# zhiyuns/AFCM

Measured on AMD Instinct MI355X. Metric: generator fwd+bwd images/sec @256^2, higher is better.
Workload: dtype bf16; 1 GPU; AFCM --model stylegan3 generator training step (fwd + L1 loss + bwd + grad all-reduce + Adam), IXI T1->T2 shape: 256x256, 4->1 channels, full-width 58.5M-param generator, random init; global_batch=16, per_gpu_batch=16, resolution=256, parallelism=dp1, world_size=1, gradient_buckets=0, comm_dtype=fp32, homogeneous_dot=True

## Files before the change

afcm_amd/_lib.py:

```python
import ctypes as C
import os

import torch

_HERE = os.path.dirname(os.path.abspath(__file__))
LIB_PATH = os.environ.get('AFCM_HIP_LIB') or os.path.join(_HERE, 'libafcm_hip.so')

F32, F16, BF16 = 0, 1, 2
E_NOKERNEL, E_INVALID = -1, -2
SIGNS_NONE, SIGNS_WRITE, SIGNS_READ = 0, 1, 2

_DTYPES = {torch.float32: F32, torch.float16: F16, torch.bfloat16: BF16}


class FilteredLReluArgs(C.Structure):
    _fields_ = [
        ('x', C.c_void_p), ('y', C.c_void_p), ('b', C.c_void_p), ('signs', C.c_void_p),
        ('fu', C.c_void_p), ('fd', C.c_void_p),
        ('dtype', C.c_int32),
        ('n', C.c_int32), ('c', C.c_int32), ('xh', C.c_int32), ('xw', C.c_int32), ('yh', C.c_int32), ('yw', C.c_int32),
        ('fuw', C.c_int32), ('fuh', C.c_int32), ('fdw', C.c_int32), ('fdh', C.c_int32),
        ('up', C.c_int32), ('down', C.c_int32),
        ('px0', C.c_int32), ('px1', C.c_int32), ('py0', C.c_int32), ('py1', C.c_int32),
        ('sx', C.c_int32), ('sy', C.c_int32), ('sh', C.c_int32), ('swb', C.c_int32),
# ... 48 lines not shown
    'afcm_filtered_lrelu': (C.c_int, [C.POINTER(FilteredLReluArgs), _vp]),
    'afcm_filtered_lrelu_workspace_bytes': (C.c_int64, []),
    'afcm_filtered_lrelu_prepare': (C.c_int, [C.POINTER(FilteredLReluArgs), _vp]),
    'afcm_filtered_lrelu_act': (C.c_int, [_vp, _vp, _i32, _i32, _i32, _i32, _i32, _i32, _i32, _i32, _i32, _f32, _f32, _f32, _i32, _vp]),
    'afcm_upfirdn2d': (C.c_int, [_vp, _vp, _vp, _i32, _i32, _i32, _i32, _i32, _i32, _i32, _i32, _i32, _i32, _i32, _i32, _i32,
                                 _i32, _i32, _i32, _f32, _vp]),
    'afcm_bias_act': (C.c_int, [_vp, _vp, _vp, _vp, _vp, _vp, _i32, _i64, _i64, _i32, _i32, _i32, _f32, _f32, _f32, _vp]),
    'afcm_conv2d_block_k': (C.c_int, [_i32]),
    'afcm_conv2d_block_k_ks': (C.c_int, [_i32, _i32]),
    'afcm_conv2d_pack_weights_bk': (C.c_int, [_vp, _vp, _i32, _i32, _i32, _i32, _i32, _i32, _i32, _vp]),
    'afcm_conv2d_pack_weights': (C.c_int, [_vp, _vp, _i32, _i32, _i32, _i32, _i32, _i32, _vp]),
    'afcm_conv2d_pack_weights2': (C.c_int, [_vp, _vp, _vp, _i32, _i32, _i32, _i32, _i32, _i32, _vp]),
    'afcm_conv2d': (C.c_int, [_vp, _vp, _vp, _vp, _vp, _i32, _i32, _i32, _i32, _i32, _i32, _i32, _i32, _i32, _vp]),
    'afcm_conv2d_ld': (C.c_int, [_vp, _vp, _vp, _vp, _vp, _i32, _i32, _i32, _i32, _i32, _i32, _i32, _i32, _i32, _i32, _i32, _vp]),
    'afcm_conv2d_plan': (C.c_int, [_i32] * 11 + [C.POINTER(_i32)]),
    'afcm_conv2d_wgrad_plan': (C.c_int, [_i32] * 11 + [C.POINTER(_i32)]),
    'afcm_conv2d_wgrad_splits': (C.c_int, [_i32, _i32, _i32, _i32]),
    'afcm_conv2d_wgrad': (C.c_int, [_vp, _vp, _vp, _vp, _i32, _i32, _i32, _i32, _i32, _i32, _i32, _i32, _vp]),
    'afcm_conv2d_wgrad_ld': (C.c_int, [_vp, _vp, _vp, _vp, _i32, _i32, _i32, _i32, _i32, _i32, _i32, _i32, _i32, _i32, _vp]),
    'afcm_conv2d_wgrad_dots_ld': (C.c_int, [_vp, _vp, _vp, _vp, _vp, _vp, _i32, _i32, _i32, _i32, _i32, _i32, _i32, _i32, _i32, _i32, _vp]),
    'afcm_scale_planes': (C.c_int, [_vp, _vp, _vp, _i32, _i32, _i64, _i32, _vp]),
    'afcm_plane_dot': (C.c_int, [_vp, _vp, _vp, _i32, _i64, _i32, _vp]),
    'afcm_plane_dot_ld': (C.c_int, [_vp, _vp, _vp, _i32, _i64, _i32, _i32, _i32, _i32, _vp]),
    'afcm_split16': (C.c_int, [_vp, _vp, _vp, _vp, _i32, _i64, _i32, _i32, _i64, _vp]),
    'afcm_conv2d_split': (C.c_int, [_vp, _vp, _vp, _vp, _vp, _i32, _i32, _i32, _i32, _i32, _i32, _i32, _i32, _i32, C.c_uint32, _i64, _vp, _vp, _vp]),
    'afcm_amax_bits': (C.c_int, [_vp, _vp, _i64, _i32, _vp, _vp]),
    'afcm_unscale': (C.c_int, [_vp, _i64, _vp, _vp, _vp]),
    'afcm_plane_dot_parts': (C.c_int, [_vp, _vp, _i64, _i32, _vp, _i32, _i64, _i32, _vp, _vp]),
    'afcm_conv2d_pack_split': (C.c_int, [_vp, _vp, _vp, _i32, _i32, _i32, _i32, _i32, _i32, C.c_uint32, _vp]),
    'afcm_plane_dot_gated_ld': (C.c_int, [_vp, _vp, _vp, _i32, _i64, _i32, _i32, _i32, _i32, _vp, _i32, _vp, _vp, _vp, _vp, _vp]),
# ... 86 lines not shown
```

afcm_amd/csrc/conv2d.hip:

```cpp
#include <stdlib.h>
#include <string.h>

#include <type_traits>

#include "conv2d_common.h"
#include "flrelu_mfma_common.h"

namespace afcm {

template <typename T> struct ConvCfg;
template <> struct ConvCfg<bf16_t> { static constexpr int BK = 16, PITCH = 24; };
template <> struct ConvCfg<f16_t>  { static constexpr int BK = 16, PITCH = 24; };
template <> struct ConvCfg<float>  { static constexpr int BK = 8,  PITCH = 9;  };

static inline int conv_bk(int dtype, int ks);
int conv2d_direct_small_cin(const void* x, void* y, const void* wp, const float* oscale, const float* obias, int dtype, int n, int cin, int cout,
                            int h, int w, int pad, int rows_pad, int bk, int ldx, int ldy, hipStream_t st);

constexpr int kPatchMax = 416;
constexpr int kPlaneX16 = 416;
constexpr int kPatchMaxX16 = kPlaneX16 - 4;
constexpr int kPatchMaxS2 = 704;
constexpr int kSlots = 256;

// ... 2 lines not shown
    void* y;
    const void* wp;
    const float* oscale;
    const float* obias;
    int N, Cin, Cout, H, W, P, Q;
    int ldx, ldy;
    int pad;
    int TH, TW, PWL, tilesX, tilesY;
    int Opad, nkc;
    int total_blocks;
    int o_base;
    unsigned magicTW;
    unsigned magicTX, magicTY, magicN, magicPC;
    int nkc_real; unsigned magicNK, term_parts; int part_bytes, last_part_bytes;
    const unsigned* bound_a; const unsigned* bound_b;
};

__host__ __device__ inline unsigned magic_u32(unsigned d) { return (unsigned)((0x100000000ull + d - 1) / d); }
__device__ __forceinline__ unsigned udiv_magic(unsigned n, unsigned magic) { return magic ? __umulhi(n, magic) : n; }

template <typename T, int BM_O, int KS>
__global__ __launch_bounds__(256, (sizeof(T) == 4 ? 1 : 2)) void conv2d_fwd_kernel(ConvParams p) {
    typedef ConvCfg<T> C;
    constexpr int BK = C::BK, PITCH = C::PITCH, MI = BM_O / 64, KK = KS * KS;
    constexpr bool F32 = sizeof(T) == 4;
    constexpr int EPV = 16 / sizeof(T);
    constexpr int PPR = BK / EPV;
    constexpr int NPIECES = KK * BM_O * PPR;
    constexpr int NWP = cdiv(NPIECES, 256);
    __shared__ __attribute__((aligned(16))) T lds[(KK * BM_O + kPatchMax) * PITCH];
// ... 213 lines not shown
            for (int reg = 0; reg < 16; reg++) ob[reg] = p.obias[min(obase + (reg & 3) + 8 * (reg >> 2), p.Cout - 1)];
        }
#pragma unroll
        for (int reg = 0; reg < 16; reg++) {
            const int o = obase + (reg & 3) + 8 * (reg >> 2);
            if (o < p.Cout) {
                T* yo = yn + (size_t)o * pq;
#pragma unroll
                for (int ti = 0; ti < 4; ti++)
                    if (poff[ti] >= 0) yo[poff[ti]] = from_f32<T>(acc[mi][ti][reg] * sc[reg] + ob[reg]);
            }
        }
    }
}

template <typename T, int BM_O, bool SPLIT = false, bool FASTEPI = false>
__global__ __launch_bounds__(256, 2) void conv2d_fwd16x_kernel(ConvParams p) {
    static_assert(sizeof(T) == 2, "16-bit types only");
    static_assert(!(SPLIT && FASTEPI), "the fp32-output epilogue has no fast form");
    typedef typename std::conditional<SPLIT, float, T>::type TO;
    constexpr int KS = 3, KK = 9, BK = 32, MO = BM_O / 32, NT = 8, BRING = MO == 4 ? 4 : 3;
    constexpr int ARING = MO == 2 ? 6 : 9;
    static_assert((KK * MO) % ARING == 0 && ARING >= 2 * MO, "static slots; a tap's fragments and the next tap's are live together");
    constexpr int PLANE_B = kPlaneX16 * 16;
    constexpr int BUF_B = 4 * PLANE_B;
    static_assert(PLANE_B % 256 == 0 && kPatchMaxX16 % 4 == 0, "planes: a multiple of 256 bytes apart, patch + sink inside");
    typedef typename std::conditional<std::is_same<T, bf16_t>::value, bf16x8, f16x8>::type frag_t;
    typedef __attribute__((ext_vector_type(4))) float f32x4;
    typedef __attribute__((ext_vector_type(4))) unsigned u32x4;
    typedef __attribute__((ext_vector_type(2))) unsigned u32x2;
    __shared__ __attribute__((aligned(256))) unsigned char lds[2 * BUF_B];

    const int tid = threadIdx.x, lane = tid & 63;
    const int wave = __builtin_amdgcn_readfirstlane(tid >> 6);
// ... 222 lines not shown
                if (has_sc) sc[mo] = __builtin_bit_cast(f32x4, __builtin_amdgcn_raw_buffer_load_b128(srs, sboff, 0, 0));
                if (has_ob) ob[mo] = __builtin_bit_cast(f32x4, __builtin_amdgcn_raw_buffer_load_b128(brs, sboff, 0, 0));
            }
            const int i16 = lane_e & 15, chalf = (lane_e >> 4) & 1, hh = lane_e >> 5;
            const int q4 = i16 >> 2, p4 = i16 & 3;
            unsigned rd_off[2];
#pragma unroll
            for (int r = 0; r < 2; r++) {
                const int prw = 8 * hh + 4 * r + q4;
                rd_off[r] = prw * EROW + (((chalf * 4 + p4) ^ ((prw >> 1) & 7)) << 3);
            }
            unsigned wr_off[2];
#pragma unroll
            for (int k = 0; k < 2; k++) wr_off[k] = (unsigned)(c16e * EROW + (((4 * k + ge) ^ ((c16e >> 1) & 7)) << 3));
            unsigned gbyte[8], gfullm = 0, slow_any = 0;
#pragma unroll
            for (int it = 0; it < (FASTEPI ? 0 : 8); it++) {
                const int j0 = wpx * 128 + (2 * it + hh) * 8;
                const int gpy = (int)__umulhi((unsigned)j0, p.magicTW), gpx = j0 - gpy * p.TW;
                const int gy = y0 + gpy, gx = x0 + gpx;
                const bool in_tile = j0 < p.TH * p.TW && gy < p.P;
                const bool valid = in_tile && gx < p.Q;
                const bool straddle = gpx + 8 > p.TW;
                const bool slow = in_tile && (straddle || (valid && gx + 8 > p.ldy));
                gbyte[it] = valid ? (unsigned)((gy * p.ldy + gx) * 2) : kGOut;
                if (!slow) gfullm |= 1u << it;
                if (__builtin_amdgcn_ballot_w64(slow) != 0) slow_any |= 1u << it;
            }
#pragma unroll
            for (int mi = 0; mi < (MO + 1) / 2; mi++) {
                const int rowbase = o0 + wo * (BM_O / 2) + mi * 32;
                const int o = rowbase + chalf * 16 + i16;
                const unsigned obyte = (o < p.Cout && mi * 32 + chalf * 16 < BM_O / 2) ? (unsigned)(o * pq * 2) : kOOut;
#pragma unroll
                for (int half = 0; half < 2; half++) {
#pragma unroll
                    for (int k = 0; k < 2; k++) {
                        const int mo = 2 * mi + k;
                        if (mo >= MO) continue;
#pragma unroll
                        for (int t4 = 0; t4 < 4; t4++) {
                            const int ti = 4 * half + t4;
                            uint2 w;
                            w.x = pack2<T>(acc[mo][ti][0] * sc[mo][0] + ob[mo][0], acc[mo][ti][1] * sc[mo][1] + ob[mo][1]);
                            w.y = pack2<T>(acc[mo][ti][2] * sc[mo][2] + ob[mo][2], acc[mo][ti][3] * sc[mo][3] + ob[mo][3]);
                            *(uint2*)(ebuf + wr_off[k] + t4 * (16 * EROW)) = w;
                        }
                    }
#pragma unroll
                    for (int i4 = 0; i4 < 4; i4++) {
                        const int it = 4 * half + i4;
                        union { s16x4 v[2]; eu32x4 q; } u;
#pragma unroll
                        for (int r = 0; r < 2; r++)
                            u.v[r] = __builtin_amdgcn_ds_read_tr16_b64_v4i16((__attribute__((address_space(3))) s16x4*)(ebuf + i4 * (16 * EROW) + rd_off[r]));
                        if constexpr (FASTEPI) {
                            const int b16 = wpx * 128 + 16 * it;
                            const int gpy = (int)__umulhi((unsigned)b16, p.magicTW), gpxs = b16 - gpy * p.TW;
                            const int gy = y0 + gpy, gxs = x0 + gpxs;
                            if (b16 < p.TH * p.TW && gy < p.P && gxs < p.Q) {
                                unsigned vo = obyte + 16u * (unsigned)hh;
                                if (gxs + 8 >= p.Q && hh) vo = kGOut;
                                __builtin_amdgcn_raw_buffer_store_b128(u.q, yrs, vo, (gy * p.ldy + gxs) * 2, 0);
                            }
                            continue;
                        }
                        const bool full = (gfullm >> it) & 1;
                        __builtin_amdgcn_raw_buffer_store_b128(u.q, yrs, full ? obyte + gbyte[it] : kGOut, 0, 0);
                        if ((slow_any >> it) & 1) {
                            if (!full) {
// ... 579 lines not shown
    }
    if (!split && x16 && rows_pad % 128 == 64 && rows_pad > 128) {
        pl.family = kConv128p64; pl.rows = 64; pl.big = rows_pad / 128;
        pl.items = tiles;
        pl.grid = conv_persistent_grid(pl.items, 3);
        return pl;
    }
    pl.family = small ? kConv64 : kConv128; pl.rows = small ? 64 : 128;
    pl.items = tiles * cdiv(cout, pl.rows);
    pl.grid = (small && (split || x16)) ? conv_persistent_grid(pl.items, 3) : pl.items;
    return pl;
}

template <typename T, int BM_O, bool SPLIT>
static int launch_fwd16x(const ConvParams& p, dim3 grid, bool fast, hipStream_t st) {
    if (!SPLIT && fast) hipLaunchKernelGGL((conv2d_fwd16x_kernel<T, BM_O, false, true>), grid, dim3(256), 0, st, p);
    else hipLaunchKernelGGL((conv2d_fwd16x_kernel<T, BM_O, SPLIT>), grid, dim3(256), 0, st, p);
    return hip_status(hipGetLastError());
}

static ConvParams conv_params(void* y, const void* x, const void* wp, const float* oscale, const float* obias, int n, int cin, int cout,
                              int h, int w, int P, int Q, int pad, int ldx, int ldy, int TH, int TW, int PWL, int rows_pad, int nkc) {
    ConvParams p;
    p.x = x; p.y = y; p.wp = wp; p.oscale = oscale; p.obias = obias;
    p.N = n; p.Cin = cin; p.Cout = cout; p.H = h; p.W = w;
    p.P = P; p.Q = Q;
    p.pad = pad;
    p.ldx = ldx; p.ldy = ldy;
    p.TH = TH; p.TW = TW; p.PWL = PWL;
    p.tilesX = cdiv(p.Q, p.TW); p.tilesY = cdiv(p.P, p.TH);
    p.magicTW = (unsigned)((0x100000000ull + (unsigned)p.TW - 1) / (unsigned)p.TW);
    p.magicTX = magic_u32((unsigned)p.tilesX); p.magicTY = magic_u32((unsigned)p.tilesY); p.magicN = magic_u32((unsigned)p.N); p.magicPC = magic_u32((unsigned)(p.PWL >> 2));
    p.Opad = rows_pad;
    p.nkc = nkc;
    p.nkc_real = p.nkc; p.magicNK = 0; p.term_parts = 0; p.part_bytes = 0; p.last_part_bytes = 0; p.bound_a = p.bound_b = nullptr; p.total_blocks = 0; p.o_base = 0;
    return p;
}

template <typename T, int BM_O>
static int launch_conv(ConvParams p, int ks, hipStream_t st, long long blocks, long long pgrid, bool fast, int o_base = 0) {
    p.o_base = o_base;
    AFCM_REQUIRE(blocks > 0 && blocks < (1ll << 31), "conv2d: grid of %lld blocks is out of range", blocks);
    dim3 grid((unsigned)blocks), block(256);
    p.total_blocks = (int)blocks;
    if constexpr (sizeof(T) == 2) {
        if (ks == 3) return launch_fwd16x<T, BM_O, false>(p, BM_O == 64 ? dim3((unsigned)pgrid) : grid, fast, st);
        hipLaunchKernelGGL((conv2d_fwd_kernel<T, BM_O, 1>), grid, block, 0, st, p);
    } else {
        if (ks == 3) hipLaunchKernelGGL((conv2d_fwd_kernel<T, BM_O, 3>), grid, block, 0, st, p);
        else hipLaunchKernelGGL((conv2d_fwd_kernel<T, BM_O, 1>), grid, block, 0, st, p);
    }
    return hip_status(hipGetLastError());
}

}

using namespace afcm;

extern "C" int afcm_conv2d_block_k(int32_t dtype) { return dtype == AFCM_F32 ? ConvCfg<float>::BK : ConvCfg<bf16_t>::BK; }
static inline int afcm::conv_bk(int dtype, int ks) { return (dtype != AFCM_F32 && ks == 3) ? 32 : afcm_conv2d_block_k(dtype); }
extern "C" int afcm_conv2d_block_k_ks(int32_t dtype, int32_t ks) { return conv_bk(dtype, ks); }

template <typename T>
static void launch_pack8(void* dst0, void* dst1, const float* w, int cout, int cin, int ks, int rows_pad0, int rows_pad1, int BK, hipStream_t st) {
    const int omax = dst0 ? rows_pad0 : round_up(cout, BK), imax = dst1 ? rows_pad1 : round_up(cin, BK);
    constexpr int BKT = ConvCfg<T>::BK;
    const int ti = BK > 16 ? PackTile<32>::TI : PackTile<BKT>::TI, to = BK > 16 ? PackTile<32>::TO : PackTile<BKT>::TO;
    dim3 grid((unsigned)cdiv(imax > cin ? imax : cin, ti), (unsigned)cdiv(omax > cout ? omax : cout, to)), block(256);
// ... 109 lines not shown
    AFCM_REQUIRE(blocks > 0 && blocks < (1ll << 31), "conv2d_stride2: grid of %lld blocks is out of range", blocks);
    AFCM_REQUIRE((long long)cin * h * w * 2ll < (1ll << 31), "conv2d_stride2: image out of range");
    if (dtype == AFCM_F16) hipLaunchKernelGGL((conv2d_fwd16s2_kernel<f16_t, 128>), dim3((unsigned)blocks), dim3(256), 0, (hipStream_t)stream, p);
    else hipLaunchKernelGGL((conv2d_fwd16s2_kernel<bf16_t, 128>), dim3((unsigned)blocks), dim3(256), 0, (hipStream_t)stream, p);
    return hip_status(hipGetLastError());
}

extern "C" int afcm_conv2d(void* y, const void* x, const void* wpacked, const float* oscale, const float* obias, int32_t dtype, int32_t n,
                           int32_t cin, int32_t cout, int32_t h, int32_t w, int32_t ks, int32_t pad, int32_t rows_pad, void* stream) {
    return afcm_conv2d_ld(y, x, wpacked, oscale, obias, dtype, n, cin, cout, h, w, ks, pad, rows_pad, 0, 0, stream);
}

extern "C" int afcm_conv2d_ld(void* y, const void* x, const void* wpacked, const float* oscale, const float* obias, int32_t dtype, int32_t n,
                              int32_t cin, int32_t cout, int32_t h, int32_t w, int32_t ks, int32_t pad, int32_t rows_pad, int32_t x_pitch,
                              int32_t y_pitch, void* stream) {
    AFCM_REQUIRE(y != nullptr && x != nullptr && wpacked != nullptr, "conv2d: null pointer");
    AFCM_REQUIRE(dtype == AFCM_F32 || dtype == AFCM_F16 || dtype == AFCM_BF16, "x must be float32, float16 or bfloat16");
    AFCM_REQUIRE(n > 0 && cin > 0 && cout > 0 && h > 0 && w > 0, "x is empty");
    AFCM_REQUIRE(ks == 1 || ks == 3, "only 1x1 and 3x3 kernels are supported");
    AFCM_REQUIRE(pad >= 0 && pad <= ks - 1, "padding must be in [0, k-1]");
    AFCM_REQUIRE(dtype == AFCM_F32 || (w % 2 == 0), "16-bit conv2d needs an even input width (got %d)", w);
    AFCM_REQUIRE(rows_pad >= cout && rows_pad % 64 == 0, "rows_pad must be a multiple of 64 covering cout");
    const int P = h + 2 * pad - ks + 1, Q = w + 2 * pad - ks + 1;
    AFCM_REQUIRE(P >= 1 && Q >= 1, "output must be at least 1x1");
    const int ldx = x_pitch ? x_pitch : w, ldy = y_pitch ? y_pitch : Q;
    if (ldx != w || ldy != Q) {
        AFCM_REQUIRE(dtype != AFCM_F32 && ks == 3, "conv2d: row pitches need the 16-bit 3x3 kernel");
        AFCM_REQUIRE(ldx >= w && ldy >= Q && ((ldx | ldy) & 1) == 0, "conv2d: row pitches %d / %d must be even and cover the widths %d / %d", ldx, ldy, w, Q);
        AFCM_REQUIRE((long long)cout * P * ldy < (1ll << 30), "conv2d: pitched output image is out of range");
    }
    AFCM_REQUIRE(dtype == AFCM_F32 || ks != 3 || (long long)cout * P * ldy * 2 < (1ll << 30), "conv2d: 16-bit output image of %lld bytes is out of range (< 2^30)", (long long)cout * P * ldy * 2);
    const ConvPlan pl = conv_plan(dtype, n, cin, cout, P, Q, ks, rows_pad, ldy, false);
    if (pl.family == kConvDirect)
        return conv2d_direct_small_cin(x, y, wpacked, oscale, obias, dtype, n, cin, cout, h, w, pad, rows_pad, 32, ldx, ldy, (hipStream_t)stream);
    ConvParams p = conv_params(y, x, wpacked, oscale, obias, n, cin, cout, h, w, P, Q, pad, ldx, ldy, pl.TH, pl.TW, pl.PWL, rows_pad, cdiv(cin, conv_bk(dtype, ks)));
    hipStream_t st = (hipStream_t)stream;
    if (pl.family == kConv96) {
        AFCM_REQUIRE(pl.items > 0 && pl.items < (1ll << 31), "conv2d: grid of %lld blocks is out of range", pl.items);
        p.total_blocks = (int)pl.items;
        const dim3 g96((unsigned)pl.grid);
        return dtype == AFCM_F16 ? launch_fwd16x<f16_t, 96, false>(p, g96, pl.fast, st) : launch_fwd16x<bf16_t, 96, false>(p, g96, pl.fast, st);
    }
    if (pl.family == kConv128p64) {
        const long long items128 = pl.items * pl.big;
        const int rc = dtype == AFCM_F16 ? launch_conv<f16_t, 128>(p, ks, st, items128, items128, pl.fast)
                                         : launch_conv<bf16_t, 128>(p, ks, st, items128, items128, pl.fast);
        if (rc != AFCM_OK) return rc;
        return dtype == AFCM_F16 ? launch_conv<f16_t, 64>(p, ks, st, pl.items, pl.grid, pl.fast, pl.big * 128)
                                 : launch_conv<bf16_t, 64>(p, ks, st, pl.items, pl.grid, pl.fast, pl.big * 128);
    }
// ... 67 lines not shown
    AFCM_REQUIRE(out != nullptr, "conv2d_plan: null pointer");
    AFCM_REQUIRE(dtype == AFCM_F32 || dtype == AFCM_F16 || dtype == AFCM_BF16, "x must be float32, float16 or bfloat16");
    AFCM_REQUIRE(n > 0 && cin > 0 && cout > 0 && h > 0 && w > 0, "x is empty");
    AFCM_REQUIRE(ks == 1 || ks == 3, "only 1x1 and 3x3 kernels are supported");
    AFCM_REQUIRE(pad >= 0 && pad <= ks - 1, "padding must be in [0, k-1]");
    AFCM_REQUIRE(!split || (ks == 3 && dtype != AFCM_F32), "conv2d_plan: the split route is 3x3 on 16-bit parts");
    const int P = h + 2 * pad - ks + 1, Q = w + 2 * pad - ks + 1;
    AFCM_REQUIRE(P >= 1 && Q >= 1, "output must be at least 1x1");
    (void)x_pitch;
    const ConvPlan pl = conv_plan(dtype, n, cin, cout, P, Q, ks, round_up(cout, 64), (!split && y_pitch) ? y_pitch : Q, split != 0);
    AFCM_REQUIRE(pl.items < (1ll << 31), "conv2d_plan: grid of %lld blocks is out of range", pl.items);
    out[0] = pl.family; out[1] = pl.rows; out[2] = pl.TH; out[3] = pl.TW; out[4] = (int32_t)pl.items; out[5] = (int32_t)pl.grid;
    out[6] = pl.fast ? 1 : 0; out[7] = pl.kernel;
    return AFCM_OK;
}
```

afcm_amd/torch_utils/ops/conv2d.py:

```python
import torch

from ... import _lib
from ... import profiling
from . import _rows


def _pad64(n):
    return (n + 63) // 64 * 64


def pack_weights(w, dtype, mode):
    lib = _lib.load()
    o, i, kh, kw = w.shape
    assert kh == kw and kh in (1, 3), 'only 1x1 and 3x3 kernels are supported'
    w = w.detach().to(torch.float32).contiguous()
    code = _lib._DTYPES[dtype]
    bk = lib.afcm_conv2d_block_k_ks(code, kh)
    rows, cols = (o, i) if mode == 0 else (i, o)
    rows_pad = _pad64(rows)
    nkc = (cols + bk - 1) // bk
    dst = torch.empty([nkc, kh * kw, rows_pad, bk], dtype=dtype, device=w.device)
    _lib.launched(lib.afcm_conv2d_pack_weights(dst.data_ptr(), w.data_ptr(), code, o, i, kh, mode, rows_pad, _lib.stream_ptr(w)),
                  'conv2d_pack_weights')
    return dst, rows_pad
# ... 279 lines not shown
    else:
        x, xld = _rows.dense(x), w
        y = torch.empty([n, cout, p, q], dtype=x.dtype, device=x.device)
    yld = q if y.is_contiguous() else y.stride(2)
    if oscale is not None:
        oscale = oscale.to(torch.float32).contiguous()
    span = profiling.span('conv2d', 2.0 * n * cout * cin * ks * ks * p * q)
    if obias is not None:
        obias = obias.to(torch.float32).contiguous()
        assert obias.numel() == cout
    _lib.launched(lib.afcm_conv2d_ld(y.data_ptr(), x.data_ptr(), wp.data_ptr(), _lib.ptr(oscale), _lib.ptr(obias), _lib.dtype_code(x), n, cin, cout, h, w,
                                     ks, pad, rows_pad, 0 if xld == w else xld, 0 if yld == q else yld, _lib.stream_ptr(x)), 'conv2d')
    if span is not None:
        span.end()
    return y


_FRAME_WGRAD_MAX = 12 << 20


def _frame_dy(dy, ks, pad):
    if ks == 3 and pad == 1 and dy.dtype in (torch.bfloat16, torch.float16) and dy.numel() <= _FRAME_WGRAD_MAX:
        return torch.nn.functional.pad(dy, [1, 1, 1, 1]), 2
    return dy, pad


def _wgrad_raw(dy, x, cout, cin, ks, pad, work_share=1.0, dots_with=None):
    lib = _lib.load()
    n, _, h, w = x.shape
    work = work_share * 2.0 * n * cout * cin * ks * ks * (h + 2 * pad - ks + 1) * (w + 2 * pad - ks + 1)
# ... 333 lines not shown
```

afcm_amd/torch_utils/ops/fused_layer.py:

```python
import torch

from ... import _lib
from . import _rows
from . import conv2d as _conv
from . import filtered_lrelu as _flr


class _ConvFilteredLRelu(torch.autograd.Function):
    @staticmethod
    def forward(ctx, x, w, in_scale, out_scale, bias, fu, fd, skip, next_scale, conv_pad, cfg, prescaled, packed=None, fork=None, link_in=None, link_out=None):
        _lib.require_gpu(x, w, in_scale, out_scale, bias, fu, fd, skip, next_scale)
        cout, cin, ks, _ = w.shape
        xs = _conv.scale_planes(x, in_scale) if (in_scale is not None and not prescaled) else x
        ctx.wpt = None
        need_wpt = ctx.needs_input_grad[0] or (ctx.needs_input_grad[2] and not prescaled)
        if packed is not None and packed[0][0].dtype == x.dtype and (packed[1] is not None or not need_wpt):
            (wp, rows_pad), ctx.wpt = packed
            bk = wp.shape[3]
            assert tuple(wp.shape) == ((cin + bk - 1) // bk, ks * ks, rows_pad, bk) and rows_pad == (cout + 63) // 64 * 64, \
                f'packed weight image {tuple(wp.shape)} does not belong to a {tuple(w.shape)} weight'
        elif need_wpt:
            (wp, rows_pad), ctx.wpt = _conv.pack_weights_both(w, x.dtype)
        else:
            wp, rows_pad = _conv.pack_weights(w, x.dtype, 0)
        y = _conv._conv_raw(xs, wp, rows_pad, out_scale, cout, ks, conv_pad, obias=bias, pitched_out=True)
        need_grad = any(ctx.needs_input_grad[:5]) or ctx.needs_input_grad[7] or ctx.needs_input_grad[8]
        keep_y = out_scale is not None and ctx.needs_input_grad[3]
        flags = [] if (keep_y and need_grad and HOMOGENEOUS_DOT) else None
        z, signs, layout, _ = _flr._run(y, fu, fd, None, None, cfg, need_grad, oscale=next_scale, skip=skip, pitched_out=True, clamp_flags_out=flags)
        flags = flags[0] if flags else None
        keep_z = (next_scale is not None and ctx.needs_input_grad[8]) or flags is not None
        ctx.save_for_backward(xs, w, in_scale, out_scale, bias, fu, fd, signs, next_scale, y if keep_y else None, z if keep_z else None,
                              flags, skip if (flags is not None and skip is not None) else None)
        ctx.skip_by_fork = False
        if fork is not None and skip is not None and next_scale is not None and ctx.needs_input_grad[7]:
            fork.scale = next_scale.detach()
            ctx.skip_by_fork = True
        ctx.link_out = link_out if (link_out is not None and next_scale is not None) else None
        if ctx.link_out is not None:
            ctx.link_out.want, ctx.link_out.gz = True, None
        ctx.link_in = link_in if (link_in is not None and prescaled) else None
        ctx.meta = (conv_pad, cfg, bool(prescaled), layout, tuple(y.shape), tuple(z.shape), skip is not None)
        return z

    @staticmethod
    @torch.autograd.function.once_differentiable
    def backward(ctx, g):
        xs, w, in_scale, out_scale, bias, fu, fd, signs, next_scale, y, z, flags, skip = ctx.saved_tensors
        conv_pad, cfg, prescaled, layout, y_shape, z_shape, has_skip = ctx.meta
        cout, cin, ks, _ = w.shape
        f32 = torch.float32
        assert g.dtype in (torch.bfloat16, torch.float16)
# ... 17 lines not shown
                dysy = _conv.plane_dot_gated(dys, y, flags, osc, gz, nsc, gsk)
            else:
                dysy = _conv.plane_dot(dys, y) if want_out else None
            db32 = torch.empty([o], dtype=f32, device=g.device) if want_db else None
            dn32 = torch.empty([n, o], dtype=f32, device=g.device) if want_next else None
            do32 = torch.empty([n, o], dtype=f32, device=g.device) if want_out else None
            b32 = None if bias is None else bias.to(f32).contiguous()
            _lib.launched(lib.afcm_layer_bwd_coefs(_lib.ptr(db32), _lib.ptr(dn32), _lib.ptr(do32), psum.data_ptr(), int(psum.shape[2]), _lib.ptr(osc),
                                                   _lib.ptr(nsc), _lib.ptr(b32), _lib.ptr(gz if want_next else None), _lib.ptr(dysy), n, o, _lib.stream_ptr(g)),
                          'layer_bwd_coefs')
            db = None if db32 is None else db32.to(bias.dtype)
            d_next = None if dn32 is None else dn32.to(next_scale.dtype)
            d_out = None if do32 is None else do32.to(out_scale.dtype)
        if has_skip and ctx.needs_input_grad[7]:
            d_skip = _conv.scale_planes(g, next_scale) if (next_scale is not None and not ctx.skip_by_fork) else g
        if ctx.needs_input_grad[0] or (ctx.needs_input_grad[2] and not prescaled):
            wpt, rows_pad = ctx.wpt if (ctx.wpt is not None and ctx.wpt[0].dtype == g.dtype) else _conv.pack_weights(w, g.dtype, 1)
            eff_in = None if prescaled else in_scale
            dx = _conv._conv_raw(dys, wpt, rows_pad, eff_in, cin, ks, ks - 1 - conv_pad, pitched_out=True)
            if ctx.needs_input_grad[2] and eff_in is not None:
                s2 = in_scale.to(f32).square()
                d_in = torch.where(s2 > 0, _conv.plane_dot(xs, dx) / s2.clamp_min(1e-30), torch.zeros_like(s2)).to(in_scale.dtype)
        if ctx.needs_input_grad[1]:
            if ctx.link_in is not None and ctx.link_in.want:
                dw, ctx.link_in.gz = _conv._wgrad_raw(dys, xs, cout, cin, ks, conv_pad, dots_with=w)
                dw = dw.to(w.dtype)
            else:
                dw = _conv._wgrad_raw(dys, xs, cout, cin, ks, conv_pad).to(w.dtype)
        return dx, dw, d_in, d_out, db, None, None, d_skip, d_next, None, None, None, None, None, None, None


HOMOGENEOUS_DOT = True



def _cfg(up, down, padding, gain, slope, clamp):
    px0, px1, py0, py1 = _flr._parse_padding(padding)
    return (int(up), int(down), px0, px1, py0, py1, float(gain), float(slope), float(clamp if clamp is not None else 'inf'), False, 0, 0, 0)


def available(x, w, fu, fd, up, down, padding, gain, slope, clamp, conv_pad):
    if w.shape[2] != 3 or x.dtype not in (torch.bfloat16, torch.float16) or x.device.type != 'cuda':
        return False
    yshape = [x.shape[0], w.shape[0], x.shape[2] + 2 * conv_pad - 2, x.shape[3] + 2 * conv_pad - 2]
    return _flr.matrix_core_available(yshape, x.dtype, x.device, fu, fd, _cfg(up, down, padding, gain, slope, clamp))


class LayerLink:
    __slots__ = ('want', 'gz')

    def __init__(self):
        self.want, self.gz = False, None


def conv_filtered_lrelu(x, w, in_scale, out_scale, bias, fu, fd, up, down, padding, gain, slope, clamp, conv_pad, skip=None,
                        next_scale=None, prescaled=False, packed=None, link_in=None, link_out=None):
    cfg = _cfg(up, down, padding, gain, slope, clamp)
    fork = getattr(skip, '_afcm_fork', None) if skip is not None else None
    return _ConvFilteredLRelu.apply(x, w, in_scale, out_scale, bias, fu, fd, skip, next_scale, int(conv_pad), cfg, bool(prescaled), packed, fork,
                                    link_in, link_out)


class _ForkState:
    __slots__ = ('scale', 'spent')

    def __init__(self):
        self.scale, self.spent = None, False


class _SkipFork(torch.autograd.Function):

    @staticmethod
    def forward(ctx, x, state):
        ctx.state = state
        return x.view_as(x), x.view_as(x)

    @staticmethod
    @torch.autograd.function.once_differentiable
    def backward(ctx, ga, gb):
        if ctx.state.spent:
            raise RuntimeError('skip_fork: the skip arm\'s style factor was consumed by an earlier backward over this graph; a second '
                               'backward (retain_graph=True) through the fused generator layers is not supported -- run the forward again')
        scale = ctx.state.scale
        ctx.state.scale, ctx.state.spent = None, scale is not None
        if gb is None:
            return ga, None
        if ga is None:
            return (gb if scale is None else _conv.scale_planes(gb, scale)), None
        out = None
        if ga.is_cuda and ga.dtype in (torch.bfloat16, torch.float16) and ga.dtype == gb.dtype and ga.shape == gb.shape:
            fa, fb = (_rows.whole_buffer(ga), _rows.whole_buffer(gb)) if not ga.is_contiguous() else (ga, gb if gb.is_contiguous() else None)
            if fa is not None and fb is not None and fa.shape == fb.shape:
                n, c, h, ld = fa.shape
                y = torch.empty_like(fa)
                sc = None if scale is None else scale.to(torch.float32).contiguous()
                rc = _lib.check(_lib.load().afcm_axpy_planes(y.data_ptr(), fa.data_ptr(), fb.data_ptr(), _lib.ptr(sc), _lib.dtype_code(fa), n * c, h * ld,
                                                            _lib.stream_ptr(fa)), 'axpy_planes')
                if rc == 0:
                    out = y[..., :ga.shape[3]]
        if out is None:
            out = ga + (gb if scale is None else _conv.scale_planes(gb, scale))
        return out, None


def skip_fork(x):
    if not (x.requires_grad and torch.is_grad_enabled()):
        return x, x
    state = _ForkState()
    a, b = _SkipFork.apply(x, state)
    b._afcm_fork = state
    return a, b
```

include/afcm_hip.h:

```cpp
#ifndef AFCM_HIP_H
#define AFCM_HIP_H

#include <stdint.h>

#ifdef __cplusplus
extern "C" {
#endif

#define AFCM_ABI_VERSION 13

enum { AFCM_F32 = 0, AFCM_F16 = 1, AFCM_BF16 = 2 };
enum { AFCM_OK = 0, AFCM_E_NOKERNEL = -1, AFCM_E_INVALID = -2 };
enum { AFCM_SIGNS_NONE = 0, AFCM_SIGNS_WRITE = 1, AFCM_SIGNS_READ = 2 };

int afcm_abi_version(void);
const char* afcm_last_error(void);
int afcm_noop(void* stream);

typedef struct afcm_filtered_lrelu_args {
    const void* x;
    void*       y;
    const void* b;
    uint8_t*    signs;
    const float* fu;
// ... 48 lines not shown

int afcm_conv2d_pack_weights2(void* dst_fwd, void* dst_dgrad, const float* w, int32_t dtype, int32_t cout, int32_t cin, int32_t ks,
                              int32_t rows_pad_fwd, int32_t rows_pad_dgrad, void* stream);
int afcm_conv2d_pack_weights_bk(void* dst, const float* w, int32_t dtype, int32_t cout, int32_t cin, int32_t ks, int32_t mode,
                                int32_t rows_pad, int32_t block_k, void* stream);

int afcm_conv2d(void* y, const void* x, const void* wpacked, const float* oscale, const float* obias, int32_t dtype, int32_t n,
                int32_t cin, int32_t cout, int32_t h, int32_t w, int32_t ks, int32_t pad, int32_t rows_pad, void* stream);
int afcm_conv2d_ld(void* y, const void* x, const void* wpacked, const float* oscale, const float* obias, int32_t dtype, int32_t n,
                   int32_t cin, int32_t cout, int32_t h, int32_t w, int32_t ks, int32_t pad, int32_t rows_pad, int32_t x_pitch,
                   int32_t y_pitch, void* stream);

int afcm_conv2d_plan(int32_t dtype, int32_t n, int32_t cin, int32_t cout, int32_t h, int32_t w, int32_t ks, int32_t pad, int32_t x_pitch,
                     int32_t y_pitch, int32_t split, int32_t out[8]);

int afcm_conv2d_wgrad_splits(int32_t n, int32_t cout, int32_t cin, int32_t p_rows);
int afcm_conv2d_wgrad(float* dw, float* workspace, const void* dy, const void* x, int32_t dtype, int32_t n, int32_t cin,
                      int32_t cout, int32_t h, int32_t w, int32_t ks, int32_t pad, void* stream);
int afcm_conv2d_wgrad_ld(float* dw, float* workspace, const void* dy, const void* x, int32_t dtype, int32_t n, int32_t cin,
                         int32_t cout, int32_t h, int32_t w, int32_t ks, int32_t pad, int32_t dy_pitch, int32_t x_pitch, void* stream);
int afcm_conv2d_wgrad_dots_ld(float* dw, float* dots, float* workspace, const void* dy, const void* x, const float* wref, int32_t dtype, int32_t n,
                              int32_t cin, int32_t cout, int32_t h, int32_t w, int32_t ks, int32_t pad, int32_t dy_pitch, int32_t x_pitch,
                              void* stream);

int afcm_conv2d_wgrad_plan(int32_t dtype, int32_t n, int32_t cin, int32_t cout, int32_t h, int32_t w, int32_t ks, int32_t pad,
                           int32_t dy_pitch, int32_t x_pitch, int32_t dots, int32_t out[8]);

int afcm_scale_planes(void* y, const void* x, const float* scale, int32_t dtype_in, int32_t dtype_out, int64_t planes,
                      int32_t hw, void* stream);

// ... 129 lines not shown
```

Baseline: 470.8 images/sec.

## Fuse skip-branch gradient add into conv dgrad epilogue

After: 472.7 images/sec, median of 2. No clear change (+0.4%).

```diff
diff --git a/afcm_amd/_lib.py b/afcm_amd/_lib.py
--- a/afcm_amd/_lib.py
+++ b/afcm_amd/_lib.py
@@ -86,6 +86,8 @@
     'afcm_conv2d': (C.c_int, [_vp, _vp, _vp, _vp, _vp, _i32, _i32, _i32, _i32, _i32, _i32, _i32, _i32, _i32, _vp]),
     'afcm_conv2d_ld': (C.c_int, [_vp, _vp, _vp, _vp, _vp, _i32, _i32, _i32, _i32, _i32, _i32, _i32, _i32, _i32, _i32, _i32, _vp]),
     'afcm_conv2d_plan': (C.c_int, [_i32] * 11 + [C.POINTER(_i32)]),
+    'afcm_conv2d_ld_epi': (C.c_int, [_vp, _vp, _vp, _vp, _vp, _i32, _i32, _i32, _i32, _i32, _i32, _i32, _i32, _i32, _i32, _i32, _vp, _vp, _vp]),
+    'afcm_conv2d_plan_epi': (C.c_int, [_i32] * 9 + [C.POINTER(_i32)]),
     'afcm_conv2d_wgrad_plan': (C.c_int, [_i32] * 11 + [C.POINTER(_i32)]),
     'afcm_conv2d_wgrad_splits': (C.c_int, [_i32, _i32, _i32, _i32]),
     'afcm_conv2d_wgrad': (C.c_int, [_vp, _vp, _vp, _vp, _i32, _i32, _i32, _i32, _i32, _i32, _i32, _i32, _vp]),
diff --git a/afcm_amd/csrc/conv2d.hip b/afcm_amd/csrc/conv2d.hip
--- a/afcm_amd/csrc/conv2d.hip
+++ b/afcm_amd/csrc/conv2d.hip
@@ -40,6 +40,7 @@
     unsigned magicTX, magicTY, magicN, magicPC;
     int nkc_real; unsigned magicNK, term_parts; int part_bytes, last_part_bytes;
     const unsigned* bound_a; const unsigned* bound_b;
+    const void* add; const float* add_scale;
 };
 
 __host__ __device__ inline unsigned magic_u32(unsigned d) { return (unsigned)((0x100000000ull + d - 1) / d); }
@@ -283,10 +284,11 @@
     }
 }
 
-template <typename T, int BM_O, bool SPLIT = false, bool FASTEPI = false>
+template <typename T, int BM_O, bool SPLIT = false, bool FASTEPI = false, bool EPI = false>
 __global__ __launch_bounds__(256, 2) void conv2d_fwd16x_kernel(ConvParams p) {
     static_assert(sizeof(T) == 2, "16-bit types only");
     static_assert(!(SPLIT && FASTEPI), "the fp32-output epilogue has no fast form");
+    static_assert(!(SPLIT && EPI), "the fp32-output epilogue has no fused form");
     typedef typename std::conditional<SPLIT, float, T>::type TO;
     constexpr int KS = 3, KK = 9, BK = 32, MO = BM_O / 32, NT = 8, BRING = MO == 4 ? 4 : 3;
     constexpr int ARING = MO == 2 ? 6 : 9;
@@ -539,6 +541,17 @@
 #pragma unroll
             for (int k = 0; k < 2; k++) wr_off[k] = (unsigned)(c16e * EROW + (((4 * k + ge) ^ ((c16e >> 1) & 7)) << 3));
             unsigned gbyte[8], gfullm = 0, slow_any = 0;
+            __amdgpu_buffer_rsrc_t adrs = yrs, asrs = srs;
+            if constexpr (EPI) {
+                adrs = __builtin_amdgcn_make_buffer_rsrc((void*)((const T*)p.add + (size_t)n * p.Cout * pq), 0, p.Cout * pq * 2, 0x00020000);
+                const bool has_as = p.add_scale != nullptr;
+                asrs = __builtin_amdgcn_make_buffer_rsrc((void*)(has_as ? p.add_scale + (size_t)n * p.Cout : (const float*)p.y), 0, has_as ? p.Cout * 4 : 0, 0x00020000);
+            }
+            auto axpy2 = [&](unsigned v, unsigned a, float s) __attribute__((always_inline)) -> unsigned {
+                union { unsigned u; T t[2]; } x, y;
+                x.u = v; y.u = a;
+                return pack2<T>(to_f32(x.t[0]) + s * to_f32(y.t[0]), to_f32(x.t[1]) + s * to_f32(y.t[1]));
+            };
 #pragma unroll
             for (int it = 0; it < (FASTEPI ? 0 : 8); it++) {
                 const int j0 = wpx * 128 + (2 * it + hh) * 8;
@@ -552,13 +565,50 @@
                 if (!slow) gfullm |= 1u << it;
                 if (__builtin_amdgcn_ballot_w64(slow) != 0) slow_any |= 1u << it;
             }
+            auto obyte_of = [&](int mi) __attribute__((always_inline)) -> unsigned {
+                const int o = o0 + wo * (BM_O / 2) + mi * 32 + chalf * 16 + i16;
+                return (o < p.Cout && mi * 32 + chalf * 16 < BM_O / 2) ? (unsigned)(o * pq * 2) : kOOut;
+            };
+            auto gaddr = [&](unsigned obyte, int it, unsigned& vo, int& so) __attribute__((always_inline)) {
+                if constexpr (FASTEPI) {
+                    const int b16 = wpx * 128 + 16 * it;
+                    const int gpy = (int)__umulhi((unsigned)b16, p.magicTW), gpxs = b16 - gpy * p.TW;
+                    const int gy = y0 + gpy, gxs = x0 + gpxs;
+                    const bool live = b16 < p.TH * p.TW && gy < p.P && gxs < p.Q;
+                    vo = (live && !(gxs + 8 >= p.Q && hh)) ? obyte + 16u * (unsigned)hh : kGOut;
+                    so = live ? (gy * p.ldy + gxs) * 2 : 0;
+                } else {
+                    vo = ((gfullm >> it) & 1) ? obyte + gbyte[it] : kGOut;
+                    so = 0;
+                }
+            };
+            constexpr int ESTAGES = 2 * ((MO + 1) / 2);
+            eu32x4 opa[2][4];
+            auto issue_ops = [&](int s) __attribute__((always_inline)) {
+                const unsigned obyte = obyte_of(s >> 1);
+#pragma unroll
+                for (int i4 = 0; i4 < 4; i4++) {
+                    unsigned vo; int so;
+                    gaddr(obyte, 4 * (s & 1) + i4, vo, so);
+                    opa[s & 1][i4] = __builtin_bit_cast(eu32x4, __builtin_amdgcn_raw_buffer_load_b128(adrs, vo, so, 0));
+                }
+            };
+            if constexpr (EPI) {
+                issue_ops(0);
+                __builtin_amdgcn_sched_barrier(0);
+            }
 #pragma unroll
             for (int mi = 0; mi < (MO + 1) / 2; mi++) {
                 const int rowbase = o0 + wo * (BM_O / 2) + mi * 32;
                 const int o = rowbase + chalf * 16 + i16;
-                const unsigned obyte = (o < p.Cout && mi * 32 + chalf * 16 < BM_O / 2) ? (unsigned)(o * pq * 2) : kOOut;
+                const unsigned obyte = obyte_of(mi);
+                float asc = 1.f;
+                if constexpr (EPI) {
+                    if (p.add_scale != nullptr) asc = __builtin_bit_cast(float, __builtin_amdgcn_raw_buffer_load_b32(asrs, (unsigned)(o * 4), 0, 0));
+                }
 #pragma unroll
                 for (int half = 0; half < 2; half++) {
+                    const int es = 2 * mi + half;
 #pragma unroll
                     for (int k = 0; k < 2; k++) {
                         const int mo = 2 * mi + k;
@@ -572,6 +622,13 @@
                             *(uint2*)(ebuf + wr_off[k] + t4 * (16 * EROW)) = w;
                         }
                     }
+                    if constexpr (EPI) {
+                        if (es + 1 < ESTAGES) {
+                            __builtin_amdgcn_sched_barrier(0);
+                            issue_ops(es + 1);
+                            __builtin_amdgcn_sched_barrier(0);
+                        }
+                    }
 #pragma unroll
                     for (int i4 = 0; i4 < 4; i4++) {
                         const int it = 4 * half + i4;
@@ -579,6 +636,30 @@
 #pragma unroll
                         for (int r = 0; r < 2; r++)
                             u.v[r] = __builtin_amdgcn_ds_read_tr16_b64_v4i16((__attribute__((address_space(3))) s16x4*)(ebuf + i4 * (16 * EROW) + rd_off[r]));
+                        if constexpr (EPI) {
+                            unsigned vo; int so;
+                            gaddr(obyte, it, vo, so);
+                            eu32x4 q;
+#pragma unroll
+                            for (int w2 = 0; w2 < 4; w2++) q[w2] = axpy2(u.q[w2], opa[es & 1][i4][w2], asc);
+                            __builtin_amdgcn_raw_buffer_store_b128(q, yrs, vo, so, 0);
+                            if constexpr (!FASTEPI) {
+                                if (((slow_any >> it) & 1) && !((gfullm >> it) & 1)) {
+                                    unsigned po[4], a32[4];
+#pragma unroll
+                                    for (int w2 = 0; w2 < 4; w2++) {
+                                        const int j = wpx * 128 + (2 * it + hh) * 8 + 2 * w2;
+                                        const int py = (int)__umulhi((unsigned)j, p.magicTW), px = j - py * p.TW;
+                                        const bool ok = j < p.TH * p.TW && y0 + py < p.P && x0 + px < p.Q;
+                                        po[w2] = ok ? obyte + (unsigned)(((y0 + py) * p.ldy + x0 + px) * 2) : kGOut;
+                                        a32[w2] = __builtin_amdgcn_raw_buffer_load_b32(adrs, po[w2], 0, 0);
+                                    }
+#pragma unroll
+                                    for (int w2 = 0; w2 < 4; w2++) __builtin_amdgcn_raw_buffer_store_b32(axpy2(u.q[w2], a32[w2], asc), yrs, po[w2], 0, 0);
+                                }
+                            }
+                            continue;
+                        }
                         if constexpr (FASTEPI) {
                             const int b16 = wpx * 128 + 16 * it;
                             const int gpy = (int)__umulhi((unsigned)b16, p.magicTW), gpxs = b16 - gpy * p.TW;
@@ -1188,6 +1269,13 @@
 
 template <typename T, int BM_O, bool SPLIT>
 static int launch_fwd16x(const ConvParams& p, dim3 grid, bool fast, hipStream_t st) {
+    if constexpr (!SPLIT && BM_O != 64) {
+        if (p.add != nullptr) {
+            if (fast) hipLaunchKernelGGL((conv2d_fwd16x_kernel<T, BM_O, false, true, true>), grid, dim3(256), 0, st, p);
+            else hipLaunchKernelGGL((conv2d_fwd16x_kernel<T, BM_O, false, false, true>), grid, dim3(256), 0, st, p);
+            return hip_status(hipGetLastError());
+        }
+    }
     if (!SPLIT && fast) hipLaunchKernelGGL((conv2d_fwd16x_kernel<T, BM_O, false, true>), grid, dim3(256), 0, st, p);
     else hipLaunchKernelGGL((conv2d_fwd16x_kernel<T, BM_O, SPLIT>), grid, dim3(256), 0, st, p);
     return hip_status(hipGetLastError());
@@ -1208,6 +1296,7 @@
     p.Opad = rows_pad;
     p.nkc = nkc;
     p.nkc_real = p.nkc; p.magicNK = 0; p.term_parts = 0; p.part_bytes = 0; p.last_part_bytes = 0; p.bound_a = p.bound_b = nullptr; p.total_blocks = 0; p.o_base = 0;
+    p.add = nullptr; p.add_scale = nullptr;
     return p;
 }
 
@@ -1226,6 +1315,8 @@
     }
     return hip_status(hipGetLastError());
 }
+
+static bool conv_has_epi(const ConvPlan& pl) { return pl.kernel == kConvKernelX16 && (pl.family == kConv128 || pl.family == kConv96); }
 
 }
 
@@ -1365,6 +1456,13 @@
 extern "C" int afcm_conv2d_ld(void* y, const void* x, const void* wpacked, const float* oscale, const float* obias, int32_t dtype, int32_t n,
                               int32_t cin, int32_t cout, int32_t h, int32_t w, int32_t ks, int32_t pad, int32_t rows_pad, int32_t x_pitch,
                               int32_t y_pitch, void* stream) {
+    return afcm_conv2d_ld_epi(y, x, wpacked, oscale, obias, dtype, n, cin, cout, h, w, ks, pad, rows_pad, x_pitch, y_pitch, nullptr, nullptr, stream);
+}
+
+extern "C" int afcm_conv2d_ld_epi(void* y, const void* x, const void* wpacked, const float* oscale, const float* obias, int32_t dtype, int32_t n,
+                                  int32_t cin, int32_t cout, int32_t h, int32_t w, int32_t ks, int32_t pad, int32_t rows_pad, int32_t x_pitch,
+                                  int32_t y_pitch, const void* add, const float* add_scale, void* stream) {
+    const bool epi = add != nullptr || add_scale != nullptr;
     AFCM_REQUIRE(y != nullptr && x != nullptr && wpacked != nullptr, "conv2d: null pointer");
     AFCM_REQUIRE(dtype == AFCM_F32 || dtype == AFCM_F16 || dtype == AFCM_BF16, "x must be float32, float16 or bfloat16");
     AFCM_REQUIRE(n > 0 && cin > 0 && cout > 0 && h > 0 && w > 0, "x is empty");
@@ -1382,9 +1480,14 @@
     }
     AFCM_REQUIRE(dtype == AFCM_F32 || ks != 3 || (long long)cout * P * ldy * 2 < (1ll << 30), "conv2d: 16-bit output image of %lld bytes is out of range (< 2^30)", (long long)cout * P * ldy * 2);
     const ConvPlan pl = conv_plan(dtype, n, cin, cout, P, Q, ks, rows_pad, ldy, false);
+    if (epi) {
+        AFCM_REQUIRE(add != nullptr, "conv2d_ld_epi: add_scale without add");
+        if (!conv_has_epi(pl)) return AFCM_E_NOKERNEL;
+    }
     if (pl.family == kConvDirect)
         return conv2d_direct_small_cin(x, y, wpacked, oscale, obias, dtype, n, cin, cout, h, w, pad, rows_pad, 32, ldx, ldy, (hipStream_t)stream);
     ConvParams p = conv_params(y, x, wpacked, oscale, obias, n, cin, cout, h, w, P, Q, pad, ldx, ldy, pl.TH, pl.TW, pl.PWL, rows_pad, cdiv(cin, conv_bk(dtype, ks)));
+    p.add = add; p.add_scale = add_scale;
     hipStream_t st = (hipStream_t)stream;
     if (pl.family == kConv96) {
         AFCM_REQUIRE(pl.items > 0 && pl.items < (1ll << 31), "conv2d: grid of %lld blocks is out of range", pl.items);
@@ -1482,3 +1585,18 @@
     out[6] = pl.fast ? 1 : 0; out[7] = pl.kernel;
     return AFCM_OK;
 }
+
+extern "C" int afcm_conv2d_plan_epi(int32_t dtype, int32_t n, int32_t cin, int32_t cout, int32_t h, int32_t w, int32_t ks, int32_t pad, int32_t y_pitch,
+                                    int32_t out[1]) {
+    AFCM_REQUIRE(out != nullptr, "conv2d_plan_epi: null pointer");
+    AFCM_REQUIRE(dtype == AFCM_F32 || dtype == AFCM_F16 || dtype == AFCM_BF16, "x must be float32, float16 or bfloat16");
+    AFCM_REQUIRE(n > 0 && cin > 0 && cout > 0 && h > 0 && w > 0, "x is empty");
+    AFCM_REQUIRE(ks == 1 || ks == 3, "only 1x1 and 3x3 kernels are supported");
+    AFCM_REQUIRE(pad >= 0 && pad <= ks - 1, "padding must be in [0, k-1]");
+    const int P = h + 2 * pad - ks + 1, Q = w + 2 * pad - ks + 1;
+    AFCM_REQUIRE(P >= 1 && Q >= 1, "output must be at least 1x1");
+    out[0] = 0;
+    if (dtype == AFCM_F32 || (w & 1)) return AFCM_OK;
+    out[0] = conv_has_epi(conv_plan(dtype, n, cin, cout, P, Q, ks, round_up(cout, 64), y_pitch ? y_pitch : Q, false)) ? 1 : 0;
+    return AFCM_OK;
+}
diff --git a/afcm_amd/torch_utils/ops/conv2d.py b/afcm_amd/torch_utils/ops/conv2d.py
--- a/afcm_amd/torch_utils/ops/conv2d.py
+++ b/afcm_amd/torch_utils/ops/conv2d.py
@@ -1,3 +1,5 @@
+import ctypes
+
 import torch
 
 from ... import _lib
@@ -317,6 +319,41 @@
     if span is not None:
         span.end()
     return y
+
+
+def _epi_operand(t, like, yld):
+    if t.dtype != like.dtype or t.shape != like.shape or t.device != like.device or _rows.pitch_of(t) != yld:
+        return False
+    return t.is_contiguous() or _rows.whole_buffer(t) is not None
+
+
+def _conv_raw_epi(x, wp, rows_pad, oscale, cout, ks, pad, add, add_scale=None):
+    if not _pitch_conv(x.dtype, ks):
+        return None
+    lib = _lib.load()
+    n, cin, h, w = x.shape
+    p, q = h + 2 * pad - ks + 1, w + 2 * pad - ks + 1
+    x, xld = _rows.rows(x)
+    y = _rows.empty([n, cout, p, q], x.dtype, x.device, pitched=True)
+    yld = q if y.is_contiguous() else y.stride(2)
+    if not _epi_operand(add, y, yld):
+        return None
+    info = (ctypes.c_int32 * 1)()
+    _lib.launched(lib.afcm_conv2d_plan_epi(_lib.dtype_code(x), n, cin, cout, h, w, ks, pad, 0 if yld == q else yld, info), 'conv2d_plan_epi')
+    if not info[0]:
+        return None
+    if oscale is not None:
+        oscale = oscale.to(torch.float32).contiguous()
+    if add_scale is not None:
+        add_scale = add_scale.to(torch.float32).contiguous()
+        assert add_scale.numel() == n * cout
+    span = profiling.span('conv2d', 2.0 * n * cout * cin * ks * ks * p * q)
+    rc = _lib.check(lib.afcm_conv2d_ld_epi(y.data_ptr(), x.data_ptr(), wp.data_ptr(), _lib.ptr(oscale), None, _lib.dtype_code(x), n, cin, cout, h, w, ks, pad,
+                                           rows_pad, 0 if xld == w else xld, 0 if yld == q else yld, add.data_ptr(), _lib.ptr(add_scale), _lib.stream_ptr(x)),
+                    'conv2d_epi')
+    if span is not None:
+        span.end()
+    return y if rc == 0 else None
 
 
 _FRAME_WGRAD_MAX = 12 << 20
diff --git a/afcm_amd/torch_utils/ops/fused_layer.py b/afcm_amd/torch_utils/ops/fused_layer.py
--- a/afcm_amd/torch_utils/ops/fused_layer.py
+++ b/afcm_amd/torch_utils/ops/fused_layer.py
@@ -8,7 +8,8 @@
 
 class _ConvFilteredLRelu(torch.autograd.Function):
     @staticmethod
-    def forward(ctx, x, w, in_scale, out_scale, bias, fu, fd, skip, next_scale, conv_pad, cfg, prescaled, packed=None, fork=None, link_in=None, link_out=None):
+    def forward(ctx, x, w, in_scale, out_scale, bias, fu, fd, skip, next_scale, conv_pad, cfg, prescaled, packed=None, fork=None, link_in=None, link_out=None,
+                fork_in=None):
         _lib.require_gpu(x, w, in_scale, out_scale, bias, fu, fd, skip, next_scale)
         cout, cin, ks, _ = w.shape
         xs = _conv.scale_planes(x, in_scale) if (in_scale is not None and not prescaled) else x
@@ -36,6 +37,8 @@
         if fork is not None and skip is not None and next_scale is not None and ctx.needs_input_grad[7]:
             fork.scale = next_scale.detach()
             ctx.skip_by_fork = True
+        ctx.fork = fork if ctx.skip_by_fork else None
+        ctx.fork_in = fork_in if ctx.needs_input_grad[0] else None
         ctx.link_out = link_out if (link_out is not None and next_scale is not None) else None
         if ctx.link_out is not None:
             ctx.link_out.want, ctx.link_out.gz = True, None
@@ -83,10 +86,19 @@
             d_out = None if do32 is None else do32.to(out_scale.dtype)
         if has_skip and ctx.needs_input_grad[7]:
             d_skip = _conv.scale_planes(g, next_scale) if (next_scale is not None and not ctx.skip_by_fork) else g
+            if ctx.skip_by_fork:
+                ctx.fork.gb = g
         if ctx.needs_input_grad[0] or (ctx.needs_input_grad[2] and not prescaled):
             wpt, rows_pad = ctx.wpt if (ctx.wpt is not None and ctx.wpt[0].dtype == g.dtype) else _conv.pack_weights(w, g.dtype, 1)
             eff_in = None if prescaled else in_scale
-            dx = _conv._conv_raw(dys, wpt, rows_pad, eff_in, cin, ks, ks - 1 - conv_pad, pitched_out=True)
+            fork = ctx.fork_in
+            if EPILOGUE_ADD and fork is not None and fork.gb is not None and not fork.spent and eff_in is None:
+                gb_buf = fork.gb if fork.gb.is_contiguous() else _rows.whole_buffer(fork.gb)
+                if gb_buf is not None and (gb_buf.shape[2] * gb_buf.shape[3]) % 8 == 0 and gb_buf.data_ptr() % 16 == 0:
+                    dx = _conv._conv_raw_epi(dys, wpt, rows_pad, None, cin, ks, ks - 1 - conv_pad, fork.gb, fork.scale)
+                    fork.folded = dx is not None
+            if dx is None:
+                dx = _conv._conv_raw(dys, wpt, rows_pad, eff_in, cin, ks, ks - 1 - conv_pad, pitched_out=True)
             if ctx.needs_input_grad[2] and eff_in is not None:
                 s2 = in_scale.to(f32).square()
                 d_in = torch.where(s2 > 0, _conv.plane_dot(xs, dx) / s2.clamp_min(1e-30), torch.zeros_like(s2)).to(in_scale.dtype)
@@ -96,11 +108,11 @@
                 dw = dw.to(w.dtype)
             else:
                 dw = _conv._wgrad_raw(dys, xs, cout, cin, ks, conv_pad).to(w.dtype)
-        return dx, dw, d_in, d_out, db, None, None, d_skip, d_next, None, None, None, None, None, None, None
+        return dx, dw, d_in, d_out, db, None, None, d_skip, d_next, None, None, None, None, None, None, None, None
 
 
 HOMOGENEOUS_DOT = True
-
+EPILOGUE_ADD = True
 
 
 def _cfg(up, down, padding, gain, slope, clamp):
@@ -127,14 +139,15 @@
     cfg = _cfg(up, down, padding, gain, slope, clamp)
     fork = getattr(skip, '_afcm_fork', None) if skip is not None else None
     return _ConvFilteredLRelu.apply(x, w, in_scale, out_scale, bias, fu, fd, skip, next_scale, int(conv_pad), cfg, bool(prescaled), packed, fork,
-                                    link_in, link_out)
+                                    link_in, link_out, getattr(x, '_afcm_fork_arm', None))
 
 
 class _ForkState:
-    __slots__ = ('scale', 'spent')
+    __slots__ = ('scale', 'spent', 'gb', 'folded')
 
     def __init__(self):
         self.scale, self.spent = None, False
+        self.gb, self.folded = None, False
 
 
 class _SkipFork(torch.autograd.Function):
@@ -151,7 +164,11 @@
             raise RuntimeError('skip_fork: the skip arm\'s style factor was consumed by an earlier backward over this graph; a second '
                                'backward (retain_graph=True) through the fused generator layers is not supported -- run the forward again')
         scale = ctx.state.scale
+        folded = ctx.state.folded
         ctx.state.scale, ctx.state.spent = None, scale is not None
+        ctx.state.gb, ctx.state.folded = None, False
+        if folded and ga is not None:
+            return ga, None
         if gb is None:
             return ga, None
         if ga is None:
@@ -178,4 +195,5 @@
     state = _ForkState()
     a, b = _SkipFork.apply(x, state)
     b._afcm_fork = state
+    a._afcm_fork_arm = state
     return a, b
diff --git a/include/afcm_hip.h b/include/afcm_hip.h
--- a/include/afcm_hip.h
+++ b/include/afcm_hip.h
@@ -86,6 +86,12 @@
 int afcm_conv2d_plan(int32_t dtype, int32_t n, int32_t cin, int32_t cout, int32_t h, int32_t w, int32_t ks, int32_t pad, int32_t x_pitch,
                      int32_t y_pitch, int32_t split, int32_t out[8]);
 
+int afcm_conv2d_ld_epi(void* y, const void* x, const void* wpacked, const float* oscale, const float* obias, int32_t dtype, int32_t n,
+                       int32_t cin, int32_t cout, int32_t h, int32_t w, int32_t ks, int32_t pad, int32_t rows_pad, int32_t x_pitch,
+                       int32_t y_pitch, const void* add, const float* add_scale, void* stream);
+int afcm_conv2d_plan_epi(int32_t dtype, int32_t n, int32_t cin, int32_t cout, int32_t h, int32_t w, int32_t ks, int32_t pad, int32_t y_pitch,
+                         int32_t out[1]);
+
 int afcm_conv2d_wgrad_splits(int32_t n, int32_t cout, int32_t cin, int32_t p_rows);
 int afcm_conv2d_wgrad(float* dw, float* workspace, const void* dy, const void* x, int32_t dtype, int32_t n, int32_t cin,
                       int32_t cout, int32_t h, int32_t w, int32_t ks, int32_t pad, void* stream);
```
